# GeekAlexis/FastMOT

Hardware: AMD Instinct MI355X
Metric: end-to-end tracker FPS @1080p/50 dets (higher is better)
Workload: dtype f16

## Files before the change

### fastmot_amd/csrc/convs.hip

```cpp
#include "net.h"
#include <cstdlib>

#ifndef FM_CONVS_PD2
#define FM_CONVS_PD2 3
#endif

namespace {

typedef float f32x16 __attribute__((ext_vector_type(16)));

#ifdef FM_CONVS_TIMING
__device__ long long g_convs_stamps[64];
#ifndef FM_CONVS_TIMING_K
#define FM_CONVS_TIMING_K 2304
#define FM_CONVS_TIMING_P 1444
#endif
#define CONVS_STAMP(i) if ((blockIdx.x == 0 || blockIdx.x == 320) && threadIdx.x == 0 && p.K == FM_CONVS_TIMING_K && p.P == FM_CONVS_TIMING_P) g_convs_stamps[(blockIdx.x ? 32 : 0) + (i)] = __builtin_readcyclecounter();
#else
#define CONVS_STAMP(i)
#endif

__device__ __attribute__((aligned(128))) f16 g_zero_page[4160];

template <int CT, int NW, int PT>
__global__ __launch_bounds__(NW * 64) void convs_kernel(const ConvParams p, int npt, int ncg) {
    constexpr int PD = PT == 2 ? FM_CONVS_PD2 : (CT == 1 ? 4 : 3);
    constexpr int BROW = 64 + 8;
    constexpr int NU = 4 * PT;
    constexpr int STAGE = NW * PT * 32 * BROW * 2, RED = NW * CT * 4 * 64 * 16;
    __shared__ __attribute__((aligned(16))) char smem[STAGE > RED ? STAGE : RED];
    const int tid = threadIdx.x, lane = tid & 63, wave = __builtin_amdgcn_readfirstlane(tid >> 6);
    const int frow = lane & 31, half = lane >> 5;
    CONVS_STAMP(0)
    const int total = npt * ncg, per_xcd = (total + 7) >> 3;
    const int logical = (blockIdx.x & 7) * per_xcd + (blockIdx.x >> 3);
    if (logical >= total) return;
    const bool weight_major = p.weight_major != 0;
    const int tile_c = weight_major ? logical / npt : logical % ncg, tile_p = weight_major ? logical % npt : logical / ncg;

    const int seg = lane & 7;
    const f16* img[NU];
    int iy0[NU], ix0[NU];
    const int hw = p.Ho * p.Wo;
    const float inv_hw = 1.f / (float)hw, inv_wo = 1.f / (float)p.Wo;
#pragma unroll
    for (int u = 0; u < NU; ++u) {
        const int pix = min(tile_p * 32 * PT + (lane >> 3) + 8 * u, p.P - 1);
        const int n = idiv_small(pix, hw, inv_hw), rem = pix - n * hw, oy = idiv_small(rem, p.Wo, inv_wo), ox = rem - oy * p.Wo;
        iy0[u] = oy * p.stride - p.pad;
        ix0[u] = ox * p.stride - p.pad - p.pad_dx;
        img[u] = p.in + (size_t)n * p.H * p.W * p.in_cs + p.in_coff + seg * 8;
    }
    f16* stage = reinterpret_cast<f16*>(smem) + wave * PT * 32 * BROW;

    const int nq = p.K >> 6;
    const int q0 = wave * nq / NW, q1 = (wave + 1) * nq / NW, nloc = q1 - q0;
    const size_t wtile = (size_t)(p.K >> 4) * 512;
    const f16* ap = p.w + ((size_t)tile_c * CT * (p.K >> 4) * 64 + lane) * 8 + (size_t)q0 * 2048;

    f16x8 fa[PD][CT][4], raw[PD][NU];
    const f16* bp[NU];
    int left = 0, kh, kw, c0;
    {
        const int k0 = q0 << 6, tap = k0 / p.Cin;
        c0 = k0 - tap * p.Cin;
        kh = tap / p.KW;
        kw = tap - kh * p.KW;
    }
    auto load = [&](int slot) {
        if (left == 0) {
#pragma unroll
            for (int u = 0; u < NU; ++u) {
                const int iy = iy0[u] + kh, ix = ix0[u] + kw;
                const bool ok = iy >= 0 && iy < p.H && ix >= 0 && ix < p.W;
                bp[u] = (ok ? img[u] + ((size_t)iy * p.W + ix) * p.in_cs : g_zero_page + seg * 8) + c0;
            }
            left = (p.Cin - c0) >> 6;
            c0 = 0;
            if (++kw == p.KW) { kw = 0; ++kh; }
        }
#pragma unroll
        for (int u = 0; u < NU; ++u) {
            raw[slot][u] = *reinterpret_cast<const f16x8*>(bp[u]);
            bp[u] += 64;
        }
#pragma unroll
        for (int i = 0; i < CT; ++i)
#pragma unroll
            for (int u = 0; u < 4; ++u) fa[slot][i][u] = *reinterpret_cast<const f16x8*>(ap + i * wtile + u * 512);
        ap += 2048;
        --left;
    };
    f32x16 acc[CT][PT];
#pragma unroll
    for (int i = 0; i < CT; ++i)
#pragma unroll
        for (int t = 0; t < PT; ++t)
#pragma unroll
            for (int r = 0; r < 16; ++r) acc[i][t][r] = 0.f;
    CONVS_STAMP(1)
#pragma unroll
    for (int r = 0; r < PD; ++r)
        if (r < nloc) load(r);
    CONVS_STAMP(2)
    for (int base = 0; base < nloc; base += PD) {
        if (base < 24) { CONVS_STAMP(8 + base) }
#pragma unroll
        for (int r = 0; r < PD; ++r) {
            if (base + r < nloc) {
#pragma unroll
                for (int u = 0; u < NU; ++u)
                    *reinterpret_cast<f16x8*>(stage + ((lane >> 3) + 8 * u) * BROW + seg * 8) = raw[r][u];
                f16x8 b[PT][4];
#pragma unroll
                for (int t = 0; t < PT; ++t)
#pragma unroll
                    for (int u = 0; u < 4; ++u)
                        b[t][u] = *reinterpret_cast<const f16x8*>(stage + (t * 32 + frow) * BROW + (u * 2 + half) * 8);
#pragma unroll
                for (int u = 0; u < 4; ++u)
#pragma unroll
                    for (int t = 0; t < PT; ++t)
#pragma unroll
                        for (int i = 0; i < CT; ++i)
                            acc[i][t] = __builtin_amdgcn_mfma_f32_32x32x16_f16(fa[r][i][u], b[t][u], acc[i][t], 0, 0, 0);
                if (base + r + PD < nloc) load(r);
            }
        }
    }
    CONVS_STAMP(3)
    __syncthreads();
    CONVS_STAMP(4)
    float4 (*red)[CT * 4][64] = reinterpret_cast<float4 (*)[CT * 4][64]>(smem);

#pragma unroll
    for (int t = 0; t < PT; ++t) {
        if (t) __syncthreads();
#pragma unroll
        for (int i = 0; i < CT; ++i)
#pragma unroll
            for (int g = 0; g < 4; ++g)
                red[wave][i * 4 + g][lane] = make_float4(acc[i][t][g * 4], acc[i][t][g * 4 + 1], acc[i][t][g * 4 + 2],
                                                         acc[i][t][g * 4 + 3]);
        __syncthreads();
        for (int e = tid; e < CT * 256; e += NW * 64) {
            const int ig = e >> 6, ln = e & 63;
            float4 a = red[0][ig][ln];
#pragma unroll
            for (int w = 1; w < NW; ++w) {
                const float4 tt = red[w][ig][ln];
                a.x += tt.x; a.y += tt.y; a.z += tt.z; a.w += tt.w;
            }
            const int co = (tile_c * CT + (ig >> 2)) * 32 + (ig & 3) * 8 + (ln >> 5) * 4;
            const long opix = ((long)tile_p * PT + t) * 32 + (ln & 31);
            if (opix >= p.P || co >= p.cout_store) continue;
            const float4 b = *reinterpret_cast<const float4*>(p.bias + co);
            float v[4] = {a.x + b.x, a.y + b.y, a.z + b.z, a.w + b.w};
            float r[4] = {0.f, 0.f, 0.f, 0.f};
            if (p.res_mode != RES_NONE) {
                const f16x4 rv = *reinterpret_cast<const f16x4*>(p.res + (size_t)opix * p.res_cs + p.res_coff + co);
#pragma unroll
                for (int j = 0; j < 4; ++j) r[j] = (float)rv[j];
            }
            if (p.res_mode == RES_BEFORE_ACT) {
#pragma unroll
                for (int j = 0; j < 4; ++j) v[j] += r[j];
            }
            apply_act_n<4>(v, p.act);
            if (p.res_mode == RES_AFTER_ACT) {
#pragma unroll
                for (int j = 0; j < 4; ++j) v[j] += r[j];
            }
            if (p.out32) {
                *reinterpret_cast<float4*>(p.out32 + (size_t)opix * p.out_cs + p.out_coff + co) = make_float4(v[0], v[1], v[2], v[3]);
            } else {
                f16x4 o;
#pragma unroll
                for (int j = 0; j < 4; ++j) o[j] = (f16)v[j];
                store_out(p, opix, co, o);
            }
        }
    }
    CONVS_STAMP(5)
#ifdef FM_CONVS_TIMING
    if ((blockIdx.x == 0 || blockIdx.x == 320) && threadIdx.x == 0 && p.K == FM_CONVS_TIMING_K && p.P == FM_CONVS_TIMING_P) { g_convs_stamps[(blockIdx.x ? 32 : 0) + 6] = nloc; g_convs_stamps[(blockIdx.x ? 32 : 0) + 7] = CT * 100 + NW * 10 + PT; }
#endif
}

template <int CT, int NW>
__global__ __launch_bounds__(NW * 64) void convs_halo_kernel(const ConvParams p, int tiles_x, int tiles_y, int ncg) {
    constexpr int PT = 2, PD = 3, TH = 8, TW = 8, HWT = TW + 2, NPOS = (TH + 2) * (TW + 2);
    extern __shared__ __attribute__((aligned(16))) char hsm[];
    f16* tile = reinterpret_cast<f16*>(hsm);
    const int ROW = p.Cin + 8;
    const int tid = threadIdx.x, lane = tid & 63, wave = __builtin_amdgcn_readfirstlane(tid >> 6);
    const int frow = lane & 31, half = lane >> 5;
    const int ntiles = tiles_x * tiles_y, total = ntiles * ncg, per_xcd = (total + 7) >> 3;
    const int logical = (blockIdx.x & 7) * per_xcd + (blockIdx.x >> 3);
    if (logical >= total) return;
    const bool weight_major = p.weight_major != 0;
    int tile_c, tile_id;
    if (weight_major) {
        tile_c = idiv_small(logical, ntiles, 1.f / (float)ntiles);
        tile_id = logical - tile_c * ntiles;
    } else {
        tile_id = idiv_small(logical, ncg, 1.f / (float)ncg);
        tile_c = logical - tile_id * ncg;
    }
    const int tyi = idiv_small(tile_id, tiles_x, 1.f / (float)tiles_x);
    const int ty0 = tyi * TH, tx0 = (tile_id - tyi * tiles_x) * TW;

    const int nq = p.K >> 6;
    const int q0 = wave * nq / NW, q1 = (wave + 1) * nq / NW, nloc = q1 - q0;
    const size_t wtile = (size_t)(p.K >> 4) * 512;
    const f16* ap = p.w + ((size_t)tile_c * CT * (p.K >> 4) * 64 + lane) * 8 + (size_t)q0 * 2048;
    f16x8 fa[PD][CT][4];
    auto load_a = [&](int slot) {
#pragma unroll
        for (int i = 0; i < CT; ++i)
#pragma unroll
            for (int u = 0; u < 4; ++u) fa[slot][i][u] = *reinterpret_cast<const f16x8*>(ap + i * wtile + u * 512);
        ap += 2048;
    };
#pragma unroll
    for (int r = 0; r < PD; ++r)
        if (r < nloc) load_a(r);

    {
        const int segs = p.Cin >> 3;
        const float inv_segs = 1.f / (float)segs;
        const f16* src = p.in + p.in_coff + (size_t)blockIdx.y * p.H * p.W * p.in_cs;
        for (int i = tid; i < NPOS * segs; i += NW * 64) {
            const int pos = idiv_small(i, segs, inv_segs), sg = i - pos * segs;
            const int py = pos / HWT, px = pos - py * HWT;
            const int iy = ty0 - 1 + py, ix = tx0 - 1 + px;
            uint4 v = make_uint4(0, 0, 0, 0);
            if (iy >= 0 && iy < p.H && ix >= 0 && ix < p.W)
                v = *reinterpret_cast<const uint4*>(src + ((size_t)iy * p.W + ix) * p.in_cs + sg * 8);
            *reinterpret_cast<uint4*>(tile + pos * ROW + sg * 8) = v;
        }
    }
    int boff[PT];
#pragma unroll
    for (int t = 0; t < PT; ++t) {
        const int pl = t * 32 + frow;
        boff[t] = ((pl >> 3) * HWT + (pl & 7)) * ROW + half * 8;
    }
    int kh, kw, c0;
    {
        const int k0 = q0 << 6, tap = k0 / p.Cin;
        c0 = k0 - tap * p.Cin;
        kh = tap / 3;
        kw = tap - kh * 3;
    }
    f32x16 acc[CT][PT];
#pragma unroll
    for (int i = 0; i < CT; ++i)
#pragma unroll
        for (int t = 0; t < PT; ++t)
#pragma unroll
            for (int r = 0; r < 16; ++r) acc[i][t][r] = 0.f;
    __syncthreads();
    for (int base = 0; base < nloc; base += PD) {
#pragma unroll
        for (int r = 0; r < PD; ++r) {
            if (base + r < nloc) {
                const int tapoff = (kh * HWT + kw) * ROW + c0;
                f16x8 b[PT][4];
#pragma unroll
                for (int t = 0; t < PT; ++t)
#pragma unroll
                    for (int u = 0; u < 4; ++u)
                        b[t][u] = *reinterpret_cast<const f16x8*>(tile + boff[t] + tapoff + u * 16);
#pragma unroll
                for (int u = 0; u < 4; ++u)
#pragma unroll
                    for (int t = 0; t < PT; ++t)
#pragma unroll
                        for (int i = 0; i < CT; ++i)
                            acc[i][t] = __builtin_amdgcn_mfma_f32_32x32x16_f16(fa[r][i][u], b[t][u], acc[i][t], 0, 0, 0);
                if (base + r + PD < nloc) load_a(r);
                c0 += 64;
                if (c0 == p.Cin) {
                    c0 = 0;
                    if (++kw == 3) { kw = 0; ++kh; }
                }
            }
        }
    }
    __syncthreads();
    float4 (*red)[CT * 4][64] = reinterpret_cast<float4 (*)[CT * 4][64]>(hsm);
#pragma unroll
    for (int t = 0; t < PT; ++t) {
        if (t) __syncthreads();
#pragma unroll
        for (int i = 0; i < CT; ++i)
#pragma unroll
            for (int g = 0; g < 4; ++g)
                red[wave][i * 4 + g][lane] = make_float4(acc[i][t][g * 4], acc[i][t][g * 4 + 1], acc[i][t][g * 4 + 2],
                                                         acc[i][t][g * 4 + 3]);
        __syncthreads();
        for (int e = tid; e < CT * 256; e += NW * 64) {
            const int ig = e >> 6, ln = e & 63;
            float4 a = red[0][ig][ln];
#pragma unroll
            for (int w = 1; w < NW; ++w) {
                const float4 tt = red[w][ig][ln];
                a.x += tt.x; a.y += tt.y; a.z += tt.z; a.w += tt.w;
            }
            const int co = (tile_c * CT + (ig >> 2)) * 32 + (ig & 3) * 8 + (ln >> 5) * 4;
            const int pl = t * 32 + (ln & 31);
            const int oy = ty0 + (pl >> 3), ox = tx0 + (pl & 7);
            if (oy >= p.Ho || ox >= p.Wo || co >= p.cout_store) continue;
            const long opix = ((long)blockIdx.y * p.Ho + oy) * p.Wo + ox;
            const float4 b = *reinterpret_cast<const float4*>(p.bias + co);
            float v[4] = {a.x + b.x, a.y + b.y, a.z + b.z, a.w + b.w};
            float r[4] = {0.f, 0.f, 0.f, 0.f};
            if (p.res_mode != RES_NONE) {
                const f16x4 rv = *reinterpret_cast<const f16x4*>(p.res + (size_t)opix * p.res_cs + p.res_coff + co);
#pragma unroll
                for (int j = 0; j < 4; ++j) r[j] = (float)rv[j];
            }
            if (p.res_mode == RES_BEFORE_ACT) {
#pragma unroll
                for (int j = 0; j < 4; ++j) v[j] += r[j];
            }
            apply_act_n<4>(v, p.act);
            if (p.res_mode == RES_AFTER_ACT) {
#pragma unroll
                for (int j = 0; j < 4; ++j) v[j] += r[j];
            }
            if (p.out32) {
                *reinterpret_cast<float4*>(p.out32 + (size_t)opix * p.out_cs + p.out_coff + co) = make_float4(v[0], v[1], v[2], v[3]);
            } else {
                f16x4 o;
#pragma unroll
                for (int j = 0; j < 4; ++j) o[j] = (f16)v[j];
                store_out(p, opix, co, o);
            }
        }
    }
}

template <int CT, int NW>
int convs_halo_launch(const ConvParams& p, int ntiles_c, hipStream_t s) {
    const int tiles_x = (p.Wo + 7) / 8, tiles_y = (p.Ho + 7) / 8, ncg = ntiles_c / CT;
    const int total = tiles_x * tiles_y * ncg;
    const size_t tile_bytes = (size_t)100 * (p.Cin + 8) * 2, red_bytes = (size_t)NW * CT * 4 * 64 * 16;
    const size_t shmem = tile_bytes > red_bytes ? tile_bytes : red_bytes;
    static size_t configured = 0;
    if (shmem > configured) {
        FM_HIP(hipFuncSetAttribute(reinterpret_cast<const void*>(convs_halo_kernel<CT, NW>),
                                   hipFuncAttributeMaxDynamicSharedMemorySize, (int)shmem));
        configured = shmem;
    }
    hipLaunchKernelGGL((convs_halo_kernel<CT, NW>), dim3(((total + 7) / 8) * 8, p.N), dim3(NW * 64), shmem, s, p, tiles_x,
                       tiles_y, ncg);
    FM_HIP(hipGetLastError());
    return 0;
}

template <int CT, int NW, int PT>
int convs_launch(const ConvParams& p, int ntiles_c, hipStream_t s) {
    const int npt = (p.P + 32 * PT - 1) / (32 * PT), ncg = ntiles_c / CT;
    const int total = npt * ncg;
    hipLaunchKernelGGL((convs_kernel<CT, NW, PT>), dim3(((total + 7) / 8) * 8), dim3(NW * 64), 0, s, p, npt, ncg);
    FM_HIP(hipGetLastError());
    return 0;
}

}

#ifdef FM_CONVS_TIMING
extern "C" int fm_debug_convs_stamps(long long* out64) {
    FM_HIP(hipDeviceSynchronize());
    FM_HIP(hipMemcpyFromSymbol(out64, HIP_SYMBOL(g_convs_stamps), sizeof(long long) * 64));
    return 0;
}
#endif

int launch_conv_streamed(const ConvParams& p_in, hipStream_t s) {
    ConvParams p = p_in;
    p.weight_major = (size_t)p.Cout * p.K >= (size_t)p.N * p.H * p.W * p.Cin ? 1 : 0;
    FM_CHECK_ARG(p.Cin % 64 == 0 && p.in_cs % 8 == 0 && p.in_coff % 8 == 0 && p.K == p.KH * p.KW * p.Cin);
    FM_CHECK_ARG(p.out_cs % 4 == 0 && p.out_coff % 4 == 0 && p.cout_store % 4 == 0 && p.Cin <= 4096);
    FM_CHECK_ARG(p.res_mode == RES_NONE || (p.res_cs % 4 == 0 && p.res_coff % 4 == 0));
    FM_CHECK_ARG(p.P < (1 << 22));
    const int ntiles_c = (p.Cout + 31) / 32, npt = ((p.batch_inv ? p.Ho * p.Wo : p.P) + 31) / 32, nq = p.K / 64;
    const bool ct2 = ntiles_c % 2 == 0 && (ntiles_c / 2) * npt >= 192;
    const bool nw8 = nq >= 16;
    constexpr int pt2_mode = 1;
    const int wgs1 = (ntiles_c / 2) * npt;
    constexpr int halo_mode = 1;
    if (halo_mode && p.KH == 3 && p.KW == 3 && p.stride == 1 && p.pad == 1 && (p.N == 1 || p.batch_inv) && p.Ho == p.H && p.Wo == p.W &&
        p.up != 2 && (size_t)100 * (p.Cin + 8) * 2 <= 150 * 1024 && nq >= 8) {
        const int tiles = ((p.Wo + 7) / 8) * ((p.Ho + 7) / 8);
        if (halo_mode == 2 || p.Ho * p.Wo * 5 >= tiles * 64 * 4) {
            if (ntiles_c % 2 == 0 && (ntiles_c / 2) * tiles >= 128) return convs_halo_launch<2, 8>(p, ntiles_c, s);
            return convs_halo_launch<1, 8>(p, ntiles_c, s);
        }
    }
    if (pt2_mode && ct2 && nq >= 16 && wgs1 > 256 && wgs1 <= 512) return convs_launch<2, 4, 2>(p, ntiles_c, s);
    if (ct2) return nw8 ? convs_launch<2, 8, 1>(p, ntiles_c, s) : convs_launch<2, 4, 1>(p, ntiles_c, s);
    return nw8 ? convs_launch<1, 8, 1>(p, ntiles_c, s) : convs_launch<1, 4, 1>(p, ntiles_c, s);
}
```

### include/fastmot_hip.h

```cpp
#ifndef FASTMOT_HIP_H
#define FASTMOT_HIP_H

#include <stddef.h>
#include <stdint.h>

#ifdef __cplusplus
extern "C" {
#endif

typedef struct fm_ctx fm_ctx;

int fm_ctx_create(int device, fm_ctx** out);
int fm_ctx_destroy(fm_ctx* ctx);
const char* fm_last_error(void);
int fm_device_count(void);
int fm_device_pci_bus_id(int device, char* buf, int buflen);
int fm_ctx_synchronize(fm_ctx* ctx);
int fm_ctx_bind_thread(fm_ctx* ctx);
int fm_ctx_set_option(fm_ctx* ctx, const char* key, int value);
int fm_ctx_get_option(fm_ctx* ctx, const char* key, int* value);
int fm_net_front_info(fm_ctx* ctx, int* k, long long* bytes, long long* passes);
int fm_trace_start(fm_ctx* ctx, int cap, int64_t* host_ns);
int fm_trace_read(fm_ctx* ctx, int cap, int32_t* tags, float* ms, int* n);
int fm_device_info(fm_ctx* ctx, char* buf, int buflen);

typedef struct fm_kf_params {
    double dt;
    double std_factor_acc, std_offset_acc;
    double std_factor_det[2], std_factor_klt[2];
    double min_std_det[2], min_std_klt[2];
    double init_pos_weight, init_vel_weight;
    double vel_coupling, vel_half_life;
} fm_kf_params;

int fm_kf_configure(fm_ctx* ctx, const fm_kf_params* p);
int fm_set_frame_rect(fm_ctx* ctx, const double tlbr[4]);

int fm_trk_create(fm_ctx* ctx, int n, const int32_t* slots, const double* det_tlbr);

int fm_trk_step(fm_ctx* ctx, int n, const int32_t* slots, const double* H,
                const double* klt_tlbr, const uint8_t* has_klt, const double* mult,
                double* tlbr_out, uint8_t* lost_out);

enum { FM_KF_WARP = 1, FM_KF_PREDICT = 2, FM_KF_UPDATE_KLT = 4 };
int fm_trk_step_ops(fm_ctx* ctx, int ops, int n, const int32_t* slots, const double* H,
                    const double* klt_tlbr, const uint8_t* has_klt, const double* mult,
                    double* tlbr_out, uint8_t* lost_out);

int fm_trk_update_det(fm_ctx* ctx, int n, const int32_t* slots, const double* det_tlbr,
                      double* tlbr_out, uint8_t* lost_out);

int fm_trk_get_state(fm_ctx* ctx, int n, const int32_t* slots, double* mean, double* cov);
int fm_trk_set_state(fm_ctx* ctx, int n, const int32_t* slots, const double* mean, const double* cov);
int fm_trk_copy_state(fm_ctx* ctx, int dst_slot, int src_slot);

int fm_feat_configure(fm_ctx* ctx, int dim);
int fm_emb_upload(fm_ctx* ctx, int n, const float* emb);
int fm_feat_update(fm_ctx* ctx, int n, const int32_t* slots, const int32_t* emb_rows);
int fm_feat_merge(fm_ctx* ctx, int dst_slot, int src_slot);
int fm_feat_reset(fm_ctx* ctx, int n, const int32_t* slots);
int fm_feat_get(fm_ctx* ctx, int slot, float* sum, float* avg, int32_t* count);
int fm_feat_read(fm_ctx* ctx, int n, const int32_t* slots, float* avg_out, int32_t* count_out);
int fm_feat_write(fm_ctx* ctx, int n, const int32_t* slots, const float* avg, const int32_t* count);

enum { FM_METRIC_EUCLIDEAN = 0, FM_METRIC_COSINE = 1 };

int fm_find_occluded(fm_ctx* ctx, int n, const double* tlbr, double thresh, uint8_t* out);

int fm_assoc_prepare(fm_ctx* ctx, int metric,
                     int nT, const int32_t* slots, const double* trk_tlbr, const int64_t* trk_label,
                     int nD, const double* det_tlbr, const int64_t* det_label,
                     const uint8_t* det_occluded, const uint8_t* trk_feat_f32);

int fm_assoc_get_pairwise(fm_ctx* ctx, double* feat, double* maha, double* iou);

enum {
    FM_STAGE_MATCHING = 0,
    FM_STAGE_IOU      = 1,
    FM_STAGE_REID     = 2
};

int fm_assoc_stage(fm_ctx* ctx, int stage, int solver,
                   int nr, const int32_t* rows, int nc, const int32_t* cols,
                   double motion_weight, double max_cost, double fill_val,
                   const int64_t* row_label_override,
                   int32_t* m_rows, int32_t* m_cols, uint8_t* match_gated, int* n_match,
                   double* cost_out);

int fm_assoc_prepare2(fm_ctx* ctx, int metric,
                      int nT, const int32_t* slots, const double* trk_tlbr, const int64_t* trk_label,
                      int nD, const double* det_tlbr, const int64_t* det_label,
                      const uint8_t* det_occluded, const uint8_t* trk_feat_f32, int after_extractor, int* host_cascade);

#define FM_CASCADE_HEADER 16
#define FM_CASCADE_PER_STAGE 1
typedef struct fm_cascade_in {
    int32_t n_groups;
    int32_t n_unconf, n_hist;
    int32_t flags;
    const int32_t* group_off;
    const int32_t* conf_rows;
    const uint8_t* conf_active;
    const int32_t* unconf_rows;
    const int32_t* hist_rows;
    const int64_t* hist_labels;
    const double* det_conf;
    double motion_weight, max_assoc_cost, fill_val, max_iou_cost, conf_thresh, max_reid_cost;
} fm_cascade_in;
int fm_assoc_cascade(fm_ctx* ctx, const fm_cascade_in* in, int32_t* out, int out_cap);
int fm_cascade_host(int nT, int nD, const double* feat, const double* maha, const double* iou,
                    const uint8_t* row_has_feat, const int64_t* trk_label, const int64_t* det_label,
                    const uint8_t* det_occluded, const fm_cascade_in* in, int32_t* out, int out_cap);
int fm_stage_cost_host(int stage, int nT, int nD, const double* feat, const double* maha, const double* iou,
                       const uint8_t* row_has_feat, const int64_t* det_label, const uint8_t* det_occluded,
                       int nr, const int32_t* rows, int nc, const int32_t* cols, const int64_t* row_labels,
                       double motion_weight, double max_cost, double fill_val, double* cost);
int fm_unmatched_order(int n, const int32_t* matched, int n_matched, int32_t* out);

int fm_lap(fm_ctx* ctx, const double* cost, int nr, int nc,
           int32_t* m_rows, int32_t* m_cols, int* n_match);
int fm_greedy(fm_ctx* ctx, const double* cost, int nr, int nc, double max_cost,
              int32_t* m_rows, int32_t* m_cols, int* n_match);
int fm_iou_dist(fm_ctx* ctx, int na, const double* a, int nb, const double* b, double* out);

enum { FM_NET_DETECTOR = 0, FM_NET_EXTRACTOR = 1,
       FM_NET_EXTRACTOR_B = 2  };
#define FM_MAX_EXTRA_EXTRACTORS 3
enum {
    FM_OP_CONV = 0,
    FM_OP_DWCONV3 = 1,
    FM_OP_MAXPOOL = 2,
    FM_OP_AVGPOOL = 3,
    FM_OP_UPSAMPLE2 = 4,
    FM_OP_COPY = 5,
    FM_OP_GATE = 6,
    FM_OP_GATE_SUM = 7,
    FM_OP_HEAD = 8,
    FM_OP_SPP = 10,
    FM_OP_LITECONV = 9,
    FM_OP_STEMCONV = 12,
    FM_OP_ADD = 13,
    FM_OP_RESBLOCK = 14,
    FM_OP_CONVS = 15,
    FM_OP_LITECHAIN = 16,
    FM_OP_CONVD = 17,
    FM_OP_STEM2 = 18,
    FM_OP_PAIR11 = 19,
    FM_OP_OSTAIL = 20,
    FM_OP_DWCONV = 21,
    FM_OP_SEPCONV = 22,
    FM_OP_POOLHEAD = 23,
    FM_OP_STEMPOOL = 24,
    FM_OP_INSTNORM = 25,
    FM_OP_CONVIN = 26,
    FM_OP_NONLOCAL = 27,
    FM_OP_GATED_SUM = 11
};
enum { FM_ACT_LINEAR = 0, FM_ACT_LEAKY = 1, FM_ACT_MISH = 2, FM_ACT_RELU = 3, FM_ACT_LOGISTIC = 4,
       FM_ACT_SWISH = 5, FM_ACT_RELU6 = 6  };
enum { FM_RES_NONE = 0, FM_RES_AFTER_ACT = 1, FM_RES_BEFORE_ACT = 2,
       FM_RES_BEFORE_NORM = 3  };

typedef struct fm_tensor {
    int32_t h, w, c;
    int32_t f32;
    int64_t offset;
} fm_tensor;

typedef struct fm_layer {
    int32_t op;
    int32_t n_in;
    int32_t in[4], in_coff[4];
    int32_t out, out_coff;
    int32_t res, res_coff, res_mode;
    int32_t cin, cout, k, stride, pad, act;
    int32_t hid;
    int32_t up;
    int32_t gate[4];
    int64_t w_off, b_off, w2_off, b2_off;
} fm_layer;

int fm_net_create(fm_ctx* ctx, int which, int max_batch, int n_tensors, const fm_tensor* tensors,
                  int n_layers, const fm_layer* layers, const void* weights, size_t weight_bytes,
                  int n_gates, int gate_channels, size_t arena_bytes);
int fm_net_destroy(fm_ctx* ctx, int which);
int fm_net_run(fm_ctx* ctx, int which, int batch);
int fm_net_tensor_write(fm_ctx* ctx, int which, int tensor, const void* host, size_t bytes);
int fm_net_tensor_read(fm_ctx* ctx, int which, int tensor, void* host, size_t bytes);
int fm_net_read_embeddings(fm_ctx* ctx, int n, float* host);
int fm_net_read_embeddings_mirror(fm_ctx* ctx, int n, float* host);
int fm_net_cost(fm_ctx* ctx, int which, int batch, double* flops, double* bytes);
int fm_net_profile(fm_ctx* ctx, int which, int batch, int iters, double* conv_ms, double* other_ms,
                   int* n_conv, int* n_other);

int fm_net_profile_layers(fm_ctx* ctx, int which, int batch, int iters, double* out);

int fm_frame_configure(fm_ctx* ctx, int width, int height, int ring_size);
int fm_frame_upload(fm_ctx* ctx, const uint8_t* bgr);
int fm_host_alloc(size_t bytes, void** out);
int fm_host_free(void* p);
int fm_frame_upload_next(fm_ctx* ctx, const uint8_t* bgr);
int fm_frame_ring_select_next(fm_ctx* ctx, int index);
int fm_frame_promote_next(fm_ctx* ctx);
int fm_detect_async_next(fm_ctx* ctx);
#define FM_MAX_DET_BATCH 4
int fm_frame_upload_ahead(fm_ctx* ctx, int k, const uint8_t* bgr);
int fm_frame_ring_select_ahead(fm_ctx* ctx, int k, int index);
int fm_detect_async_ahead(fm_ctx* ctx, int n);
int fm_frame_ring_store(fm_ctx* ctx, int index, const uint8_t* bgr);
int fm_frame_ring_select(fm_ctx* ctx, int index);
int fm_frame_read(fm_ctx* ctx, uint8_t* bgr);
#define FM_NV12_BT601 0
#define FM_NV12_BT709 1
int fm_frame_upload_nv12(fm_ctx* ctx, const uint8_t* y, const uint8_t* uv, int pitch, int matrix);
int fm_frame_upload_ahead_nv12(fm_ctx* ctx, int k, const uint8_t* y, const uint8_t* uv, int pitch, int matrix);
int fm_frame_ring_store_nv12(fm_ctx* ctx, int index, const uint8_t* y, const uint8_t* uv, int pitch, int matrix);

#define FM_ERR_UNSUPPORTED (-4)
#define FM_JPEG_UNSUPPORTED_PROGRESSIVE 1
#define FM_JPEG_UNSUPPORTED_ARITHMETIC 2
#define FM_JPEG_UNSUPPORTED_PROCESS 3
#define FM_JPEG_UNSUPPORTED_PRECISION 4
#define FM_JPEG_UNSUPPORTED_COMPONENTS 5
#define FM_JPEG_UNSUPPORTED_COLORSPACE 6
#define FM_JPEG_UNSUPPORTED_SAMPLING 7
#define FM_JPEG_UNSUPPORTED_SCANS 8
struct fm_jpeg_info {
    int32_t width, height;
    int32_t ncomp;
    int32_t hsamp[3], vsamp[3];
    int32_t mcu_w, mcu_h;
    int32_t mcus_x, mcus_y;
    int32_t restart_interval;
    int32_t blocks_w[3], blocks_h[3];
    int32_t unsupported;
    int64_t coef_offset[3];
    int64_t coef_count;
};
int fm_jpeg_info(const uint8_t* data, size_t n, struct fm_jpeg_info* out);
int fm_jpeg_entropy_decode(const uint8_t* data, size_t n, const struct fm_jpeg_info* info, int16_t* coef, uint16_t* qt);
int fm_frame_upload_jpeg(fm_ctx* ctx, const struct fm_jpeg_info* info, const int16_t* coef, const uint16_t* qt);
int fm_frame_upload_ahead_jpeg(fm_ctx* ctx, int k, const struct fm_jpeg_info* info, const int16_t* coef, const uint16_t* qt);
int fm_frame_ring_store_jpeg(fm_ctx* ctx, int index, const struct fm_jpeg_info* info, const int16_t* coef, const uint16_t* qt);

#define FM_SRC_BGR 0
#define FM_SRC_NV12 1
#define FM_SRC_JPEG 2
#define FM_SRC_MAX_DIM 16384
struct fm_frame_src {
    int32_t kind, width, height;
    const uint8_t* bgr;
    const uint8_t *y, *uv;
    int32_t pitch, matrix;
    const struct fm_jpeg_info* info;
    const int16_t* coef;
    const uint16_t* qt;
};
int fm_frame_upload_src(fm_ctx* ctx, const struct fm_frame_src* src);
int fm_frame_upload_ahead_src(fm_ctx* ctx, int k, const struct fm_frame_src* src);
int fm_frame_ring_store_src(fm_ctx* ctx, int index, const struct fm_frame_src* src);

#define FM_YUV_420 0
#define FM_YUV_422 1
#define FM_YUV_444 2
#define FM_YUV_MONO 3
struct fm_frame_planar {
    int32_t width, height, chroma, matrix;
    const uint8_t *y, *u, *v;
    int32_t pitch_y, pitch_c;
};
int fm_frame_upload_planar(fm_ctx* ctx, const struct fm_frame_planar* f);
int fm_frame_upload_ahead_planar(fm_ctx* ctx, int k, const struct fm_frame_planar* f);
int fm_frame_ring_store_planar(fm_ctx* ctx, int index, const struct fm_frame_planar* f);

#define FM_PACKED_RGB 0
#define FM_PACKED_BGR 1
#define FM_PACKED_RGBX 2
#define FM_PACKED_BGRX 3
#define FM_PACKED_XRGB 4
#define FM_PACKED_XBGR 5
#define FM_PACKED_YUY2 6
#define FM_PACKED_UYVY 7
#define FM_PACKED_YVYU 8
#define FM_PACKED_BT601 0
#define FM_PACKED_BT709 1
#define FM_PACKED_BT601_FULL 16
#define FM_PACKED_BT709_FULL 17
struct fm_frame_packed {
    int32_t format, width, height, pitch, matrix;
    const uint8_t* data;
};
int fm_frame_upload_packed(fm_ctx* ctx, const struct fm_frame_packed* f);
int fm_frame_upload_ahead_packed(fm_ctx* ctx, int k, const struct fm_frame_packed* f);
int fm_frame_ring_store_packed(fm_ctx* ctx, int index, const struct fm_frame_packed* f);

#define FM_BAYER_RGGB 0
#define FM_BAYER_GRBG 1
#define FM_BAYER_GBRG 2
#define FM_BAYER_BGGR 3
#define FM_BAYER_BILINEAR 0
#define FM_BAYER_MHC 1
struct fm_frame_bayer {
    int32_t pattern, width, height, pitch, depth, method, black, gain_r, gain_g, gain_b;
    const uint8_t* data;
};
int fm_frame_upload_bayer(fm_ctx* ctx, const struct fm_frame_bayer* f);
int fm_frame_upload_ahead_bayer(fm_ctx* ctx, int k, const struct fm_frame_bayer* f);
int fm_frame_ring_store_bayer(fm_ctx* ctx, int index, const struct fm_frame_bayer* f);

#define FM_DEEP_PLANAR 0
#define FM_DEEP_SEMIPLANAR 1
#define FM_DEEP_BT601 0
#define FM_DEEP_BT709 1
#define FM_DEEP_BT2020 2
struct fm_frame_deep {
    int32_t width, height, chroma, matrix, depth, layout;
    const uint8_t *y, *u, *v;
    int32_t pitch_y, pitch_c;
};
int fm_frame_upload_deep(fm_ctx* ctx, const struct fm_frame_deep* f);
int fm_frame_upload_ahead_deep(fm_ctx* ctx, int k, const struct fm_frame_deep* f);
int fm_frame_ring_store_deep(fm_ctx* ctx, int index, const struct fm_frame_deep* f);

#define FM_DEV_HWC 0
#define FM_DEV_CHW 1
#define FM_DEV_NV12 2
#define FM_DEV_U8 0
#define FM_DEV_F16 1
#define FM_DEV_F32 2
#define FM_DEV_ORDER_RGB 0
#define FM_DEV_ORDER_BGR 1
#define FM_DEV_READY 1
#define FM_DEV_TICKETS 16
struct fm_frame_device {
    const void* plane[3];
    int64_t     pitch[3];
    int32_t     width, height;
    int32_t     layout;
    int32_t     dtype;
    int32_t     format;
    int32_t     matrix;
    float       scale;
    void*       stream;
    int32_t     flags;
};
int fm_frame_upload_device(fm_ctx* ctx, const struct fm_frame_device* f);
int fm_frame_upload_ahead_device(fm_ctx* ctx, int k, const struct fm_frame_device* f, uint64_t* ticket);
int fm_frame_ring_store_device(fm_ctx* ctx, int index, const struct fm_frame_device* f);
int fm_frame_device_done(fm_ctx* ctx, uint64_t ticket, int wait);
int fm_frame_device_check(const struct fm_frame_device* f);

int fm_frame_remap_set(fm_ctx* ctx, int src_w, int src_h, const int32_t* xy, const uint8_t border_bgr[3]);
int fm_frame_remap_clear(fm_ctx* ctx);
int fm_remap_bgr_host(const uint8_t* src, int src_w, int src_h, const int32_t* xy, uint8_t* dst, int width, int height,
                      const uint8_t border_bgr[3]);

size_t fm_jpeg_encode_bound(int width, int height);
int fm_jpeg_encode_tables(int quality, uint16_t* qt);
int fm_jpeg_encode_header(int width, int height, int quality, uint8_t* out, size_t capacity, size_t* length);
int fm_jpeg_encode_assemble(int width, int height, int quality, const uint32_t* seg_len, const uint8_t* segs, size_t segs_bytes,
                            uint8_t* out, size_t capacity, size_t* length);
int fm_frame_encode_jpeg(fm_ctx* ctx, int quality, uint8_t* out, size_t capacity, size_t* length);
int fm_jpeg_encode_bgr(fm_ctx* ctx, const uint8_t* pixels, int width, int height, size_t pitch, int quality, uint8_t* out,
                       size_t capacity, size_t* length);
int fm_jpeg_encode_stream_ms(fm_ctx* ctx, float* ms);

#define FM_OVL_RECT_FILL 0
#define FM_OVL_RECT_OUTLINE 1
#define FM_OVL_LINE 2
#define FM_OVL_DOT 3
#define FM_OVL_MASK 4
#define FM_OVERLAY_MAX_CMDS 65536
#define FM_OVERLAY_MAX_MASK_BYTES (4u << 20)
#define FM_OVERLAY_MAX_COORD (1 << 20)
typedef struct fm_overlay_cmd {
    int32_t kind;
    int32_t x0, y0, x1, y1;
    uint8_t b, g, r;
    uint8_t thickness;
    uint32_t mask_off;
    int32_t reserved;
} fm_overlay_cmd;
int fm_overlay_check(const fm_overlay_cmd* cmds, int n, const uint8_t* masks, size_t mask_bytes, int width, int height);
int fm_overlay_render_host(uint8_t* pixels, int width, int height, size_t pitch, const fm_overlay_cmd* cmds, int n,
                           const uint8_t* masks, size_t mask_bytes);
int fm_frame_render_overlay(fm_ctx* ctx, const fm_overlay_cmd* cmds, int n, const uint8_t* masks, size_t mask_bytes);
int fm_overlay_read(fm_ctx* ctx, uint8_t* out);
int fm_overlay_encode_jpeg(fm_ctx* ctx, int quality, uint8_t* out, size_t capacity, size_t* length);
int fm_overlay_stream_ms(fm_ctx* ctx, float* ms);

#define FM_REDACT_PIXELATE 0
#define FM_REDACT_SMOOTH 1
#define FM_REDACT_FILL 2
#define FM_REDACT_RECT 0
#define FM_REDACT_ELLIPSE 1
#define FM_REDACT_MAX_REGIONS 4096
#define FM_REDACT_MAX_CELLS (1 << 20)
typedef struct fm_redact_region {
    int32_t x0, y0, x1, y1;
    int32_t mode;
    int32_t shape;
    int32_t cell;
    uint8_t b, g, r;
    uint8_t reserved;
} fm_redact_region;
int fm_redact_check(const fm_redact_region* regions, int n, int width, int height);
int fm_redact_render_host(uint8_t* pixels, int width, int height, size_t pitch, const fm_redact_region* regions, int n);
int fm_frame_render_redacted(fm_ctx* ctx, const fm_redact_region* regions, int n_regions, const fm_overlay_cmd* cmds, int n_cmds,
                             const uint8_t* masks, size_t mask_bytes);
int fm_redact_stream_ms(fm_ctx* ctx, float* ms);

#define FM_EXPORT_FRAME 0
#define FM_EXPORT_OVERLAY 1
size_t fm_i420_bound(int width, int height);
int fm_frame_export_i420(fm_ctx* ctx, int which, uint8_t* out, size_t capacity, size_t* length);
int fm_i420_from_bgr(fm_ctx* ctx, const uint8_t* pixels, int width, int height, size_t pitch, uint8_t* out, size_t capacity,
                     size_t* length);

#define FM_OBJENC_MAX_REGIONS 1024
#define FM_OBJENC_MAX_MCUS 16384
typedef struct fm_crop_rect {
    int32_t x0, y0, x1, y1;
} fm_crop_rect;
typedef struct fm_crop_plan {
    int32_t width, height;
    int32_t mcus_x, mcus_y;
    int32_t first_mcu, first_block, first_row;
    int32_t reserved;
    uint64_t raw_offset;
    uint64_t bound;
} fm_crop_plan;
typedef struct fm_crop_totals {
    int32_t mcus, blocks, rows;
    int32_t reserved;
    uint64_t raw_bytes;
    uint64_t bound;
} fm_crop_totals;
size_t fm_jpeg_encode_regions_bound(const fm_crop_rect* rects, int n, int shrink);
int fm_jpeg_encode_regions_plan(const fm_crop_rect* rects, int n, int shrink, fm_crop_plan* plans, fm_crop_totals* totals);
int fm_jpeg_encode_regions_assemble(const fm_crop_plan* plans, int n, int quality, const uint32_t* seg_len, const uint8_t* segs,
                                    size_t segs_bytes, uint8_t* out, size_t capacity, size_t* offsets);
int fm_frame_encode_regions(fm_ctx* ctx, int which, const fm_crop_rect* rects, int n, int shrink, int quality, uint8_t* out,
                            size_t capacity, size_t* offsets);

#define FM_MAX_HEADS 4
#define FM_MAX_ANCHORS 6
typedef struct fm_det48 {
    double tlbr[4];
    int64_t label;
    double conf;
} fm_det48;

typedef struct fm_yolo_cfg {
    int32_t in_w, in_h;
    int32_t roi_x, roi_y, roi_w, roi_h;
    int32_t input_tensor;
    int32_t n_heads;
    int32_t head_tensor[FM_MAX_HEADS];
    int32_t grid_w[FM_MAX_HEADS], grid_h[FM_MAX_HEADS], n_anchors[FM_MAX_HEADS];
    float anchors[FM_MAX_HEADS][2 * FM_MAX_ANCHORS];
    float scale_xy[FM_MAX_HEADS];
    int32_t num_classes, new_coords;
    uint8_t label_mask[128];
    double conf_thresh, nms_thresh, max_area, min_aspect_ratio;
    double size[2], offset[2];
    int32_t max_candidates;
} fm_yolo_cfg;

int fm_detect_configure(fm_ctx* ctx, const fm_yolo_cfg* cfg);
int fm_detect_async(fm_ctx* ctx);
int fm_detect_sync(fm_ctx* ctx, fm_det48* out, int cap, int* n);
int fm_detect_last_counts(fm_ctx* ctx, int* n_candidates, int* n_detections);
int fm_detect_preprocess_only(fm_ctx* ctx);
int fm_filter_dets(fm_ctx* ctx, const float* rows, int n, fm_det48* out, int cap, int* n_out);
int fm_detect_raw_candidates(fm_ctx* ctx, float* rows, int cap, int* n);
int fm_detect_net_ms(fm_ctx* ctx, float* ms);
int fm_detect_configure_tiles(fm_ctx* ctx, int n_tiles, const int32_t* origins, int region_w, int region_h,
                              const double* offsets, double merge_thresh);
int fm_detect_last_tiles(fm_ctx* ctx, fm_det48* out, int cap, int32_t* counts, int* n_tiles);
int fm_detect_merge_tiles(const fm_det48* dets, const int32_t* tile_ids, int n, int n_tiles, double thresh,
                          fm_det48* out, int* n_out);

int fm_extract_configure(fm_ctx* ctx, int input_tensor, int in_w, int in_h);
int fm_extract_async(fm_ctx* ctx, int n, const double* tlbr);
int fm_extract_sync(fm_ctx* ctx, int n, float* emb);
int fm_extract_read_input(fm_ctx* ctx, int n, float* out);

typedef struct fm_flow_cfg {
    int32_t small_w, small_h;
    int32_t bg_w, bg_h;
    int32_t win_size, max_level, max_count;
    double epsilon;
    int32_t fast_thresh;
    int32_t max_corners, block_size;
    double quality_level;
    int32_t gray_coeff_bits;
} fm_flow_cfg;
int fm_flow_configure(fm_ctx* ctx, const fm_flow_cfg* cfg);
int fm_flow_init(fm_ctx* ctx);
int fm_flow_begin(fm_ctx* ctx);
int fm_flow_targets(fm_ctx* ctx, int nT, const double* inside_tlbr, const float* kps, const int32_t* kp_off,
                    int32_t* area_out, uint8_t* keep_out);
int fm_flow_detect(fm_ctx* ctx, int n, const int32_t* track_idx, const double* track_tlbr,
                   const int32_t* min_dist, int cap, float* pts_out, int32_t* counts_out);
int fm_flow_background(fm_ctx* ctx, int cap, float* pts_out, int* n_out);
int fm_flow_prepare(fm_ctx* ctx, int nT, const double* inside_tlbr, const double* full_tlbr,
                    const float* kps, const int32_t* kp_off, double feat_density, double feat_dist_factor,
                    int32_t* area_out, uint8_t* keep_out, uint8_t* needy_out, int pts_cap,
                    float* new_pts_out, int32_t* new_off_out, int32_t* new_cnt_out, int* n_new_out,
                    int bg_cap, float* bg_pts_out, int* n_bg_out);
int fm_flow_lk(fm_ctx* ctx, int n, const float* prev_pts, float* next_pts, uint8_t* status, float* err);
int fm_flow_swap(fm_ctx* ctx);
int fm_flow_estimate(fm_ctx* ctx, int n_pts, const float* prev_pts, const float* cur_pts,
                     const uint8_t* status, int nT, const int32_t* begins, const int32_t* ends,
                     int bg_begin, int bg_end, const double* track_tlbr, int frame_w, int frame_h,
                     int ransac_max_iter, double ransac_conf, int inlier_thresh,
                     double* H_out, int* ok_out, int32_t* result_out, double* est_tlbr_out,
                     int32_t* n_matched_out, uint8_t* inlier_out);
typedef struct fm_flow_predict_params {
    double feat_density, feat_dist_factor;
    float opt_scale[2], bg_scale[2];
    double max_error;
    int32_t ransac_max_iter;
    double ransac_conf;
    int32_t inlier_thresh;
    int32_t frame_w, frame_h;
} fm_flow_predict_params;
enum { FM_FLOW_OK = 0, FM_FLOW_NO_BACKGROUND = 1, FM_FLOW_NO_HOMOGRAPHY = 2 };
int fm_flow_predict(fm_ctx* ctx, int nT, const double* inside_tlbr, const double* full_tlbr, const float* kps,
                    const int32_t* kp_off, const fm_flow_predict_params* prm, int pts_cap, float* prev_out,
                    float* cur_out, int32_t* trk_off_out, int32_t* bg_range_out, double* H_out, int* status_out,
                    int32_t* result_out, double* est_tlbr_out, int32_t* n_matched_out);
int fm_track_predict_async(fm_ctx* ctx, int nT, const double* inside_tlbr, const double* full_tlbr, const float* kps,
                           const int32_t* kp_off, const fm_flow_predict_params* prm, int pts_cap, float* prev_out,
                           float* cur_out, int32_t* trk_off_out, int32_t* bg_range_out, double* H_out,
                           int32_t* result_out, double* est_tlbr_out, int32_t* n_matched_out, int nK,
                           const int32_t* slots, const int32_t* ages, const int32_t* sorted_idx, double age_penalty,
                           double* tlbr_out, uint8_t* lost_out);
int fm_track_predict_wait(fm_ctx* ctx, int* status_out, int* kalman_done_out);
#define FM_MAX_SSD_TILES 16
#define FM_MAX_SSD_HEADS 6
typedef struct fm_ssd_cfg {
    int32_t input_tensor, in_w, in_h;
    int32_t n_heads;
    int32_t head_tensor[FM_MAX_SSD_HEADS], map_w[FM_MAX_SSD_HEADS], map_h[FM_MAX_SSD_HEADS], n_anchors[FM_MAX_SSD_HEADS];
    const float* anchors;
    int32_t n_anchor_rows;
    float box_scales[4];
    int32_t num_classes;
    int32_t topk;
    float nms_thresh;
    int32_t n_tiles;
    int32_t tile_x[FM_MAX_SSD_TILES], tile_y[FM_MAX_SSD_TILES];
    int32_t region_w, region_h;
} fm_ssd_cfg;
int fm_ssd_configure(fm_ctx* ctx, const fm_ssd_cfg* cfg);
int fm_ssd_detect_async(fm_ctx* ctx);
int fm_ssd_detect_sync(fm_ctx* ctx, float* rows, int cap, int* n);
int fm_ssd_preprocess_only(fm_ctx* ctx);
int fm_ssd_stage_ms(fm_ctx* ctx, float ms[3]);
int fm_ssd_postprocess_host_heads(fm_ctx* ctx, const float* const* heads, float* rows, int cap, int* n);

size_t fm_litechain_lds_bytes(int c, int w, int h);
int fm_resblock_supported(int c, int mid);
int fm_sepconv_supported(int cin, int cout, int stride);
int fm_convin_supported(int K, int cout, int hw);
int fm_nonlocal_supported(int c, int hw);
int fm_flow_timing(double* out5, int reset);
int fm_flow_read_image(fm_ctx* ctx, int which, uint8_t* out, int* w, int* h);

int fm_gallery_unique_id(char* out128);
int fm_gallery_init(fm_ctx* ctx, int channel, int world, int rank, const char* id128, size_t row_bytes);
int fm_gallery_allgather_async(fm_ctx* ctx, int channel, const void* send_row);
int fm_gallery_allgather_wait(fm_ctx* ctx, int channel, void* recv_rows, float* stream_ms_out);
int fm_gallery_destroy(fm_ctx* ctx, int channel);

#ifdef __cplusplus
}
#endif
#endif
```

Baseline: 1072.

## Add row-band LDS-staged implicit-GEMM kernel for 3x3 same convolutions

Adds a convs_rows kernel that stages the full input row band (pixel run plus one-row halo) for a 3x3 stride-1 conv into LDS once, then reads all nine taps from LDS while streaming weights through registers, with a cross-wave reduction at the end. It is enabled by default through an env-controlled mode and is chosen for shapes that miss the existing halo and PT2 paths when the band fits in the device LDS limit. The aim is to cut repeated global input loads for these convs, at the cost of large dynamic LDS use and lower occupancy.

Result: faster. 1087 (median of 6 runs) (+1.5%).

```diff
diff --git a/fastmot_amd/csrc/convs.hip b/fastmot_amd/csrc/convs.hip
--- a/fastmot_amd/csrc/convs.hip
+++ b/fastmot_amd/csrc/convs.hip
@@ -1,4 +1,6 @@
 #include "net.h"
+#include <algorithm>
+#include <atomic>
 #include <cstdlib>
 
 #ifndef FM_CONVS_PD2
@@ -16,8 +18,11 @@
 #define FM_CONVS_TIMING_P 1444
 #endif
 #define CONVS_STAMP(i) if ((blockIdx.x == 0 || blockIdx.x == 320) && threadIdx.x == 0 && p.K == FM_CONVS_TIMING_K && p.P == FM_CONVS_TIMING_P) g_convs_stamps[(blockIdx.x ? 32 : 0) + (i)] = __builtin_readcyclecounter();
+__device__ long long g_rows_stamps[8][16];
+#define ROWS_STAMP(i) if ((blockIdx.x & 31) == 0 && blockIdx.x < 256 && threadIdx.x == 0 && p.K == 4608 && p.Cout == 1024) g_rows_stamps[blockIdx.x >> 5][i] = wall_clock64();
 #else
 #define CONVS_STAMP(i)
+#define ROWS_STAMP(i)
 #endif
 
 __device__ __attribute__((aligned(128))) f16 g_zero_page[4160];
@@ -342,6 +347,184 @@
     }
 }
 
+template <int CT, int NW, int PT>
+__global__ __launch_bounds__(NW * 64) void convs_rows_kernel(const ConvParams p, int runs, int ncg) {
+    constexpr int PD = 3, FU = 4;
+    extern __shared__ __attribute__((aligned(16))) char hsm[];
+    f16* tile = reinterpret_cast<f16*>(hsm);
+    const int ROW = p.Cin + 8;
+    const int tid = threadIdx.x, lane = tid & 63, wave = __builtin_amdgcn_readfirstlane(tid >> 6);
+    const int frow = lane & 31, half = lane >> 5;
+    const int total = runs * ncg, per_xcd = (total + 7) >> 3;
+    const int logical = (blockIdx.x & 7) * per_xcd + (blockIdx.x >> 3);
+    if (logical >= total) return;
+    ROWS_STAMP(0)
+    const bool weight_major = p.weight_major != 0;
+    int tile_c, run;
+    if (weight_major) {
+        tile_c = idiv_small(logical, runs, 1.f / (float)runs);
+        run = logical - tile_c * runs;
+    } else {
+        run = idiv_small(logical, ncg, 1.f / (float)ncg);
+        tile_c = logical - run * ncg;
+    }
+    const int hw = p.Ho * p.Wo, WT = p.W + 2;
+    const float inv_w = 1.f / (float)p.Wo, inv_wt = 1.f / (float)WT;
+    const int first = run * 32 * PT, last = min(first + 32 * PT, hw) - 1;
+    const int oy0 = idiv_small(first, p.Wo, inv_w), oy1 = idiv_small(last, p.Wo, inv_w);
+    const int pos0 = first - oy0 * p.Wo, pos1 = (oy1 - oy0 + 2) * WT + last - oy1 * p.Wo + 2;
+
+    const int nq = p.K >> 6;
+    const int q0 = wave * nq / NW, q1 = (wave + 1) * nq / NW, nloc = q1 - q0;
+    const size_t wtile = (size_t)(p.K >> 4) * 512;
+    const f16* ap = p.w + ((size_t)tile_c * CT * (p.K >> 4) * 64 + lane) * 8 + (size_t)q0 * 2048;
+    f16x8 fa[PD][CT][4];
+    auto load_a = [&](int slot) {
+#pragma unroll
+        for (int i = 0; i < CT; ++i)
+#pragma unroll
+            for (int u = 0; u < 4; ++u) fa[slot][i][u] = *reinterpret_cast<const f16x8*>(ap + i * wtile + u * 512);
+        ap += 2048;
+    };
+#pragma unroll
+    for (int r = 0; r < PD; ++r)
+        if (r < nloc) load_a(r);
+    ROWS_STAMP(1)
+
+    {
+        const int segs = p.Cin >> 3, items = (pos1 - pos0 + 1) * segs;
+        const float inv_segs = 1.f / (float)segs;
+        const f16* src = p.in + p.in_coff + (size_t)blockIdx.y * p.H * p.W * p.in_cs;
+        for (int i0 = tid; i0 < items; i0 += FU * NW * 64) {
+            uint4 v[FU];
+#pragma unroll
+            for (int j = 0; j < FU; ++j) {
+                const int i = i0 + j * NW * 64;
+                v[j] = make_uint4(0, 0, 0, 0);
+                if (i < items) {
+                    const int q = idiv_small(i, segs, inv_segs), sg = i - q * segs, pos = pos0 + q;
+                    const int py = idiv_small(pos, WT, inv_wt);
+                    const int iy = oy0 - 1 + py, ix = pos - py * WT - 1;
+                    if (iy >= 0 && iy < p.H && ix >= 0 && ix < p.W)
+                        v[j] = *reinterpret_cast<const uint4*>(src + ((size_t)iy * p.W + ix) * p.in_cs + sg * 8);
+                }
+            }
+            ROWS_STAMP(2)
+#pragma unroll
+            for (int j = 0; j < FU; ++j) {
+                const int i = i0 + j * NW * 64;
+                if (i < items) {
+                    const int q = idiv_small(i, segs, inv_segs);
+                    *reinterpret_cast<uint4*>(tile + (pos0 + q) * ROW + (i - q * segs) * 8) = v[j];
+                }
+            }
+        }
+    }
+    ROWS_STAMP(3)
+    int boff[PT];
+#pragma unroll
+    for (int t = 0; t < PT; ++t) {
+        const int pix = min(first + t * 32 + frow, hw - 1);
+        const int oy = idiv_small(pix, p.Wo, inv_w);
+        boff[t] = ((oy - oy0) * WT + pix - oy * p.Wo) * ROW + half * 8;
+    }
+    int kh, kw, c0;
+    {
+        const int k0 = q0 << 6, tap = k0 / p.Cin;
+        c0 = k0 - tap * p.Cin;
+        kh = tap / 3;
+        kw = tap - kh * 3;
+    }
+    f32x16 acc[CT][PT];
+#pragma unroll
+    for (int i = 0; i < CT; ++i)
+#pragma unroll
+        for (int t = 0; t < PT; ++t)
+#pragma unroll
+            for (int r = 0; r < 16; ++r) acc[i][t][r] = 0.f;
+    __syncthreads();
+    ROWS_STAMP(4)
+    for (int base = 0; base < nloc; base += PD) {
+#pragma unroll
+        for (int r = 0; r < PD; ++r) {
+            if (base + r < nloc) {
+                const int tapoff = (kh * WT + kw) * ROW + c0;
+                f16x8 b[PT][4];
+#pragma unroll
+                for (int t = 0; t < PT; ++t)
+#pragma unroll
+                    for (int u = 0; u < 4; ++u)
+                        b[t][u] = *reinterpret_cast<const f16x8*>(tile + boff[t] + tapoff + u * 16);
+#pragma unroll
+                for (int u = 0; u < 4; ++u)
+#pragma unroll
+                    for (int t = 0; t < PT; ++t)
+#pragma unroll
+                        for (int i = 0; i < CT; ++i)
+                            acc[i][t] = __builtin_amdgcn_mfma_f32_32x32x16_f16(fa[r][i][u], b[t][u], acc[i][t], 0, 0, 0);
+                if (base + r + PD < nloc) load_a(r);
+                c0 += 64;
+                if (c0 == p.Cin) {
+                    c0 = 0;
+                    if (++kw == 3) { kw = 0; ++kh; }
+                }
+            }
+        }
+    }
+    ROWS_STAMP(5)
+    __syncthreads();
+    ROWS_STAMP(6)
+    float4 (*red)[NW][CT * 4][64] = reinterpret_cast<float4 (*)[NW][CT * 4][64]>(hsm);
+#pragma unroll
+    for (int t = 0; t < PT; ++t)
+#pragma unroll
+        for (int i = 0; i < CT; ++i)
+#pragma unroll
+            for (int g = 0; g < 4; ++g)
+                red[t][wave][i * 4 + g][lane] = make_float4(acc[i][t][g * 4], acc[i][t][g * 4 + 1], acc[i][t][g * 4 + 2],
+                                                            acc[i][t][g * 4 + 3]);
+    __syncthreads();
+    for (int e = tid; e < PT * CT * 256; e += NW * 64) {
+        const int t = e / (CT * 256), ig = (e >> 6) % (CT * 4), ln = e & 63;
+        float4 a = red[t][0][ig][ln];
+#pragma unroll
+        for (int w = 1; w < NW; ++w) {
+            const float4 tt = red[t][w][ig][ln];
+            a.x += tt.x; a.y += tt.y; a.z += tt.z; a.w += tt.w;
+        }
+        const int co = (tile_c * CT + (ig >> 2)) * 32 + (ig & 3) * 8 + (ln >> 5) * 4;
+        const int pix = first + t * 32 + (ln & 31);
+        if (pix >= hw || co >= p.cout_store) continue;
+        const long opix = (long)blockIdx.y * hw + pix;
+        const float4 b = *reinterpret_cast<const float4*>(p.bias + co);
+        float v[4] = {a.x + b.x, a.y + b.y, a.z + b.z, a.w + b.w};
+        float r[4] = {0.f, 0.f, 0.f, 0.f};
+        if (p.res_mode != RES_NONE) {
+            const f16x4 rv = *reinterpret_cast<const f16x4*>(p.res + (size_t)opix * p.res_cs + p.res_coff + co);
+#pragma unroll
+            for (int j = 0; j < 4; ++j) r[j] = (float)rv[j];
+        }
+        if (p.res_mode == RES_BEFORE_ACT) {
+#pragma unroll
+            for (int j = 0; j < 4; ++j) v[j] += r[j];
+        }
+        apply_act_n<4>(v, p.act);
+        if (p.res_mode == RES_AFTER_ACT) {
+#pragma unroll
+            for (int j = 0; j < 4; ++j) v[j] += r[j];
+        }
+        if (p.out32) {
+            *reinterpret_cast<float4*>(p.out32 + (size_t)opix * p.out_cs + p.out_coff + co) = make_float4(v[0], v[1], v[2], v[3]);
+        } else {
+            f16x4 o;
+#pragma unroll
+            for (int j = 0; j < 4; ++j) o[j] = (f16)v[j];
+            store_out(p, opix, co, o);
+        }
+    }
+    ROWS_STAMP(7)
+}
+
 template <int CT, int NW>
 int convs_halo_launch(const ConvParams& p, int ntiles_c, hipStream_t s) {
     const int tiles_x = (p.Wo + 7) / 8, tiles_y = (p.Ho + 7) / 8, ncg = ntiles_c / CT;
@@ -360,6 +543,89 @@
     return 0;
 }
 
+int g_convs_rows = -1;
+
+int convs_rows_mode() {
+    if (g_convs_rows < 0) {
+        const char* e = getenv("FASTMOT_CONVS_ROWS");
+        g_convs_rows = e ? atoi(e) : 1;
+    }
+    return g_convs_rows;
+}
+
+int convs_rows_tile_rows(int hw, int W, int PT) {
+    int rows = 0;
+    for (int first = 0; first < hw; first += 32 * PT) {
+        const int last = (first + 32 * PT < hw ? first + 32 * PT : hw) - 1;
+        rows = std::max(rows, last / W - first / W + 3);
+    }
+    return rows;
+}
+
+size_t convs_rows_tile_bytes(int H, int W, int Cin, int PT) {
+    return (size_t)convs_rows_tile_rows(H * W, W, PT) * (W + 2) * (Cin + 8) * 2;
+}
+
+int convs_rows_choice(bool same, int H, int W, int Cin, int Cout, size_t lds_limit, int mode) {
+    const int ntiles_c = (Cout + 31) / 32, hw = H * W, npt = (hw + 31) / 32, nq = 9 * Cin / 64;
+    if (!mode || !same || Cin % 64 || nq < 16) return 0;
+    const int wgs1 = (ntiles_c / 2) * npt;
+    if (ntiles_c % 2 == 0 && wgs1 > 256 && wgs1 <= 512) return 0;
+    if (mode == 1 && 100 * (size_t)(Cin + 8) * 2 <= 150 * 1024 && hw * 5 >= ((W + 7) / 8) * ((H + 7) / 8) * 64 * 4)
+        return 0;
+    const bool fits1 = convs_rows_tile_bytes(H, W, Cin, 1) <= lds_limit, fits2 = convs_rows_tile_bytes(H, W, Cin, 2) <= lds_limit;
+    if (mode > 2) {
+        const int pt = mode / 10, ct = mode % 10 == 2 && ntiles_c % 2 == 0 ? 2 : 1;
+        return (pt == 1 && fits1) || (pt == 2 && fits2) ? pt * 10 + ct : 0;
+    }
+    const int runs1 = npt, runs2 = (hw + 63) / 64;
+    if (fits2 && ntiles_c * runs2 >= 192) return 21;
+    if (fits1 && ntiles_c % 2 == 0 && (ntiles_c / 2) * runs1 >= 192) return 12;
+    return fits1 ? 11 : 0;
+}
+
+bool convs_rows_shape(const ConvParams& p) {
+    return p.KH == 3 && p.KW == 3 && p.stride == 1 && p.pad == 1 && p.pad_dx == 0 && (p.N == 1 || p.batch_inv) && p.Ho == p.H &&
+           p.Wo == p.W && p.up != 2 && p.K == 9 * p.Cin;
+}
+
+int convs_device_lds(size_t* limit) {
+    static std::atomic<int> known[64];
+    int dev = 0, v = 0;
+    FM_HIP(hipGetDevice(&dev));
+    if (dev < 64 && (v = known[dev].load(std::memory_order_relaxed)) > 0) {
+        *limit = (size_t)v;
+        return 0;
+    }
+    int optin = 0;
+    FM_HIP(hipDeviceGetAttribute(&v, hipDeviceAttributeMaxSharedMemoryPerBlock, dev));
+    if (hipDeviceGetAttribute(&optin, hipDeviceAttributeSharedMemPerBlockOptin, dev) != hipSuccess) (void)hipGetLastError();
+    v = std::max(v, optin);
+    if (dev < 64) known[dev].store(v, std::memory_order_relaxed);
+    *limit = (size_t)v;
+    return 0;
+}
+
+template <int CT, int NW, int PT>
+int convs_rows_launch(const ConvParams& p, int ntiles_c, size_t lds_limit, hipStream_t s) {
+    const int runs = (p.Ho * p.Wo + 32 * PT - 1) / (32 * PT), ncg = ntiles_c / CT;
+    const int total = runs * ncg;
+    const size_t tile_bytes = convs_rows_tile_bytes(p.H, p.W, p.Cin, PT), red_bytes = (size_t)PT * NW * CT * 4 * 64 * 16;
+    const size_t shmem = tile_bytes > red_bytes ? tile_bytes : red_bytes;
+    FM_CHECK_ARG(shmem <= lds_limit);
+    static std::atomic<unsigned long long> configured{0};
+    int dev = 0;
+    FM_HIP(hipGetDevice(&dev));
+    if (dev >= 64 || !(configured.load(std::memory_order_relaxed) >> dev & 1)) {
+        FM_HIP(hipFuncSetAttribute(reinterpret_cast<const void*>(convs_rows_kernel<CT, NW, PT>),
+                                   hipFuncAttributeMaxDynamicSharedMemorySize, (int)lds_limit));
+        if (dev < 64) configured.fetch_or(1ull << dev, std::memory_order_relaxed);
+    }
+    hipLaunchKernelGGL((convs_rows_kernel<CT, NW, PT>), dim3(((total + 7) / 8) * 8, p.N), dim3(NW * 64), shmem, s, p, runs, ncg);
+    FM_HIP(hipGetLastError());
+    return 0;
+}
+
 template <int CT, int NW, int PT>
 int convs_launch(const ConvParams& p, int ntiles_c, hipStream_t s) {
     const int npt = (p.P + 32 * PT - 1) / (32 * PT), ncg = ntiles_c / CT;
@@ -375,6 +641,11 @@
 extern "C" int fm_debug_convs_stamps(long long* out64) {
     FM_HIP(hipDeviceSynchronize());
     FM_HIP(hipMemcpyFromSymbol(out64, HIP_SYMBOL(g_convs_stamps), sizeof(long long) * 64));
+    return 0;
+}
+extern "C" int fm_debug_rows_stamps(long long* out128) {
+    FM_HIP(hipDeviceSynchronize());
+    FM_HIP(hipMemcpyFromSymbol(out128, HIP_SYMBOL(g_rows_stamps), sizeof(long long) * 128));
     return 0;
 }
 #endif
@@ -391,6 +662,17 @@
     const bool nw8 = nq >= 16;
     constexpr int pt2_mode = 1;
     const int wgs1 = (ntiles_c / 2) * npt;
+    if (const int mode = convs_rows_mode(); mode && convs_rows_shape(p)) {
+        size_t lds_limit = 0;
+        if (int err = convs_device_lds(&lds_limit)) return err;
+        switch (convs_rows_choice(true, p.H, p.W, p.Cin, p.Cout, lds_limit, mode)) {
+            case 21: return convs_rows_launch<1, 8, 2>(p, ntiles_c, lds_limit, s);
+            case 22: return convs_rows_launch<2, 8, 2>(p, ntiles_c, lds_limit, s);
+            case 12: return convs_rows_launch<2, 8, 1>(p, ntiles_c, lds_limit, s);
+            case 11: return convs_rows_launch<1, 8, 1>(p, ntiles_c, lds_limit, s);
+            default: break;
+        }
+    }
     constexpr int halo_mode = 1;
     if (halo_mode && p.KH == 3 && p.KW == 3 && p.stride == 1 && p.pad == 1 && (p.N == 1 || p.batch_inv) && p.Ho == p.H && p.Wo == p.W &&
         p.up != 2 && (size_t)100 * (p.Cin + 8) * 2 <= 150 * 1024 && nq >= 8) {
@@ -404,3 +686,15 @@
     if (ct2) return nw8 ? convs_launch<2, 8, 1>(p, ntiles_c, s) : convs_launch<2, 4, 1>(p, ntiles_c, s);
     return nw8 ? convs_launch<1, 8, 1>(p, ntiles_c, s) : convs_launch<1, 4, 1>(p, ntiles_c, s);
 }
+
+extern "C" int fm_convs_rows_supported(int cin, int cout, int k, int stride, int h, int w, int up, int lds_limit, int mode) {
+    const int ho = (h + 2 * (k / 2) - k) / stride + 1, wo = (w + 2 * (k / 2) - k) / stride + 1;
+    const bool same = k == 3 && stride == 1 && ho == h && wo == w && up != 2;
+    return cin > 0 && cout > 0 && h > 0 && w > 0 && lds_limit > 0 ? convs_rows_choice(same, h, w, cin, cout, (size_t)lds_limit, mode) : 0;
+}
+
+extern "C" int fm_convs_rows_set(int mode) {
+    FM_CHECK_ARG(mode == 0 || mode == 1 || mode == 2 || mode == 11 || mode == 12 || mode == 21 || mode == 22);
+    g_convs_rows = mode;
+    return 0;
+}
diff --git a/include/fastmot_hip.h b/include/fastmot_hip.h
--- a/include/fastmot_hip.h
+++ b/include/fastmot_hip.h
@@ -563,6 +563,8 @@
 
 size_t fm_litechain_lds_bytes(int c, int w, int h);
 int fm_resblock_supported(int c, int mid);
+int fm_convs_rows_supported(int cin, int cout, int k, int stride, int h, int w, int up, int lds_limit, int mode);
+int fm_convs_rows_set(int mode);
 int fm_sepconv_supported(int cin, int cout, int stride);
 int fm_convin_supported(int K, int cout, int hw);
 int fm_nonlocal_supported(int c, int hw);
```
